# okieraised/rs-face-detection

Hardware: AMD Instinct MI355X
Metric: images/sec + p50 latency, RetinaFace-R50 640x640 b32 (end-to-end detect: preprocess + CNN + decode + NMS; `value` = frames resident in HBM, `value_host_path` = SURVEY 8(d)'s H2D -> ... -> D2H figure) (higher is better)
Workload: dtype bf16; 1 GPU; RetinaFace-ResNet50 640x640 batch=32 bf16 per GPU (BASELINE.json configs[2]); batch_per_gpu=32, global_batch=32, max_det=1024, parallelism=single GPU

## Files before the change

include/rfd.h:

```cpp
#ifndef RFD_H
#define RFD_H

#include <stddef.h>
#include <stdint.h>

#ifdef __cplusplus
extern "C" {
#endif

#define RFD_VERSION 1

#if defined(__GNUC__)
#define RFD_API __attribute__((visibility("default")))
#else
#define RFD_API
#endif

typedef enum rfd_status {
    RFD_OK = 0,
    RFD_ERR_INVALID_ARG = -1,
    RFD_ERR_NO_DEVICE = -2,
    RFD_ERR_HIP = -3,
    RFD_ERR_CAPACITY = -4,
    RFD_ERR_STATE = -5,
// ... 584 lines not shown
                                    const rfd_redact_config *cfg , int32_t *applied , int async);
RFD_API int rfd_redact_faces(rfd_ctx *ctx, const rfd_image *imgs, const rfd_image *dst, int n, const rfd_dets *dets, const uint32_t *sel,
                             const rfd_redact_config *cfg, int32_t *applied);

RFD_API int rfd_get_stats(rfd_ctx *ctx, rfd_stats *stats);
RFD_API int rfd_get_config(const rfd_ctx *ctx, rfd_config *cfg);
RFD_API int rfd_set_thresholds(rfd_ctx *ctx, float confidence_threshold, float iou_threshold);
RFD_API int rfd_set_profiling(rfd_ctx *ctx, int enable);
RFD_API int rfd_get_conv_profile(rfd_ctx *ctx, float *ms_conv, double *flops_conv, int *launches);
RFD_API int rfd_get_op_profile(rfd_ctx *ctx, float *ms, int cap);

RFD_API int rfd_debug_tensor_io(rfd_ctx *ctx, int tensor_id, int n, void *host, int write);
RFD_API int rfd_debug_run_ops(rfd_ctx *ctx, int n, int first_op, int last_op);
RFD_API int rfd_debug_run_chain(rfd_ctx *ctx, int n, int first_op, int last_op, int batch_off, int co_running);
RFD_API int rfd_debug_pass_chains(rfd_ctx *ctx, int n, int *sizes, int cap);
RFD_API int rfd_debug_buffer_io(rfd_ctx *ctx, int tensor_id, void *host, size_t bytes, int write, size_t *image_pitch);
RFD_API int rfd_debug_set_conv_tile(rfd_ctx *ctx, int tile);
RFD_API int rfd_debug_op_kernels(rfd_ctx *ctx, int n, int op, int co_running, char *names, int cap);
RFD_API int rfd_debug_op_kernels_static(int backbone, int net_w, int net_h, int n, int op, int co_running, int tile, int schedule,
                                        int cus, char *names, int cap);
RFD_API int rfd_debug_set_concurrency(rfd_ctx *ctx, int multi_stream, int split_min_part, int split_max_parts,
                                      int use_graph);

RFD_API int rfd_debug_poke_nms_flag(rfd_ctx *ctx, int value);
RFD_API int rfd_debug_align_setup(rfd_ctx *ctx, int n, const float *boxes, const float *kps, const int32_t *found,
                                  const int32_t *img_w, const int32_t *img_h, const rfd_alignment_config *cfg, int32_t *mode,
                                  double *M, int32_t *roi, double *scale, int32_t *area_fast);
RFD_API int rfd_debug_persistent_kernel(int i, const char **name, size_t *lds_bytes);

#ifdef __cplusplus
// ... 4 lines not shown
```

rs-face-detection_amd/csrc/detector.hip:

```cpp
#include <dlfcn.h>
#include <stdarg.h>
#include <stdlib.h>

#include <algorithm>
#include <cmath>
#include <memory>
#include <mutex>
#include <vector>

#include "ctx_access.h"
#include "face_host.h"
#include "frame_host.h"
#include "host_resources.h"
#include "jpeg_encode_host.h"
#include "jpeg_host.h"
#include "network.h"
#include "redact_host.h"
#include "shot_quality_host.h"
#include "view_plan.h"

namespace rfd {

static thread_local char g_err[512] = "";

// ... 151 lines not shown
    JpegEncoder encoder;
    Redact redact;
    struct PipeSlot {
        DevBuf frames, imgs, scale, ob, ol, oc, ot;
        Pinned<PreImage> pin_imgs;
        Pinned<float> pin_scale, h_ob, h_ol;
        Pinned<int> h_oc, h_ot;
        Event h2d, done, post;
        int n = 0;
    };
    static constexpr int kPipe = 2;
    static constexpr int kPipeRows = 128;
    PipeSlot pipe[kPipe];
    int pipe_head = 0, pipe_tail = 0, pipe_inflight = 0;
    DevBuf ov_imgs[2], ov_scale[2];
    Event ov_chain_done[2][2], ov_post_done[2], ov_desc;
    bool ov_post_valid[2] = {false, false};
    int ov_parity = 0;
    int ov_last_n = -1;
    Event ov_resync;
    Rccl::Comm comm = nullptr;
    int comm_rank = 0, comm_world = 0;
    rfd_stats stats;
    float conv_ms = 0.f;
    double conv_flops = 0.0;
    int conv_launches = 0;

    int ensure_network()
    {
        if (net_created) return RFD_OK;
        RFD_TRY(net.create(cfg.backbone, cfg.image_w, cfg.image_h, cfg.max_batch_size, cfg.precision, cfg.schedule));
// ... 229 lines not shown
        c->conv_ms = 0.f; c->conv_flops = 0.0; c->conv_launches = 0;
        for (size_t i = 0; i < c->net.g.ops.size(); ++i)
            if (c->net.g.ops[i].kind == OP_CONV || c->net.g.ops[i].kind == OP_B2B) {
                c->conv_ms += c->net.op_ms[i];
                c->conv_flops += 2.0 * c->net.g.layer_macs((int)i) * n;
                ++c->conv_launches;
            }
    }
    return RFD_OK;
}

int detect_overlapped(rfd_ctx *c, const rfd_image *imgs, int n, rfd_dets *out, hipEvent_t frames_ready = nullptr)
{
    Network &net = c->net;
    RFD_TRY(net.ensure_alt_heads());
    const size_t B = (size_t)c->cfg.max_batch_size;
    if (!c->ov_desc) {
        RFD_TRY(c->ov_desc.create());
        RFD_TRY(c->ov_resync.create());
        for (int a = 0; a < 2; ++a) {
            RFD_TRY(c->ov_post_done[a].create());
            for (int b = 0; b < 2; ++b) RFD_TRY(c->ov_chain_done[a][b].create());
            RFD_TRY(c->ov_imgs[a].reserve(B * sizeof(PreImage)));
            RFD_TRY(c->ov_scale[a].reserve(B * sizeof(float)));
        }
    }
    const int par = (c->ov_parity ^= 1);
    PreImage *pis;
    float *pin_scales;
    RFD_TRY(acquire_frame_slot(c, &pis, &pin_scales));
    for (int i = 0; i < n; ++i) RFD_TRY(fill_pre_image(c, imgs[i], i, &pis[i], &pin_scales[i]));
    RFD_TRY(place_frames(c, imgs, n, true, pis, sizeof *pis));
    hipStream_t st[2] = {net.part_stream[0], net.part_stream[1]};
    if (c->ov_last_n != n) {
        RFD_HIP(hipEventRecord(c->ov_resync, c->stream));
        for (int p = 0; p < 2; ++p) RFD_HIP(hipStreamWaitEvent(st[p], c->ov_resync, 0));
    }
    c->ov_last_n = n;
    if (frames_ready)
        for (int p = 0; p < 2; ++p) RFD_HIP(hipStreamWaitEvent(st[p], frames_ready, 0));
    if (c->ov_post_valid[par])
        for (int p = 0; p < 2; ++p) RFD_HIP(hipStreamWaitEvent(st[p], c->ov_post_done[par], 0));
    RFD_HIP(hipMemcpyAsync(c->ov_imgs[par].p, pis, n * sizeof(PreImage), hipMemcpyHostToDevice, st[0]));
    RFD_HIP(hipMemcpyAsync(c->ov_scale[par].p, pin_scales, n * sizeof(float), hipMemcpyHostToDevice, st[0]));
    RFD_TRY(c->frame_ring.record(st[0]));
    RFD_HIP(hipEventRecord(c->ov_desc, st[0]));
    RFD_HIP(hipStreamWaitEvent(st[1], c->ov_desc, 0));
    net.head_parity = par;
    net.co_running = 1;
    int chain[Network::kMaxParts];
    if (net.pass_chains(n, chain) != 2) { set_error("overlapped calls run as two chains"); return RFD_ERR_STATE; }
    const int B0 = chain[0];
    int status = RFD_OK;
    for (int p = 0; p < 2 && status == RFD_OK; ++p) {
        const int off = p ? B0 : 0, Bp = chain[p];
        status = launch_preprocess(pre_params(c, (const PreImage *)c->ov_imgs[par].p + off, off), Bp, st[p]);
        if (status == RFD_OK) status = net.run(Bp, st[p], 0, -1, off, p);
        if (status == RFD_OK && hipEventRecord(c->ov_chain_done[par][p], st[p]) != hipSuccess) status = RFD_ERR_HIP;
    }
    net.co_running = 0;
    if (status != RFD_OK) { net.head_parity = 0; c->ov_last_n = -1; return status; }
    for (int p = 0; p < 2; ++p) RFD_HIP(hipStreamWaitEvent(c->stream, c->ov_chain_done[par][p], 0));
    DecodeParams dp = decode_params(c, true);
    net.head_parity = 0;
    RFD_TRY(post_network(c, dp, false, n, out->boxes, out->landmarks, out->count, out->total, nullptr,
                         (const float *)c->ov_scale[par].p));
    RFD_HIP(hipEventRecord(c->ov_post_done[par], c->stream));
    c->ov_post_valid[par] = true;
    return RFD_OK;
}

int detect_impl(rfd_ctx *c, const rfd_image *imgs, int n, rfd_dets *out, bool on_device, int async, bool frames_on_device)
{
    RFD_CHECK_ARG(c != nullptr, "ctx is null");
    RFD_CHECK_ARG(out && out->boxes && out->landmarks && out->count, "output buffers are null");
    RFD_TRY(check_images(c, imgs, n));
    RFD_TRY(c->ensure_network());
    if (!c->net.weights_ready) { set_error("network weights are not initialised"); return RFD_ERR_STATE; }
    if (async == 2 && on_device && frames_on_device && !c->net.profiling && c->net.multi_stream && c->net.num_parts(n) == 2) {
// ... 910 lines not shown
    RFD_HIP(hipSetDevice(c->cfg.device_id));
    const float *scales;
    RFD_TRY(stage_frames(c, imgs, n, false, &scales));
    const size_t npix = (size_t)n * c->cfg.image_h * c->cfg.image_w;
    PreParams pp = pre_params(c, c->imgs.p, -1);
    if (det_img) { RFD_TRY(c->scratch[0].reserve(npix * 3)); pp.out_det_img = (uint8_t *)c->scratch[0].p; }
    if (tensor) { RFD_TRY(c->scratch[1].reserve(npix * 3 * sizeof(float))); pp.out_tensor = (float *)c->scratch[1].p; }
    RFD_TRY(launch_preprocess(pp, n, c->stream));
    if (det_img) RFD_HIP(hipMemcpyAsync(det_img, pp.out_det_img, npix * 3, hipMemcpyDeviceToHost, c->stream));
    if (tensor) RFD_HIP(hipMemcpyAsync(tensor, pp.out_tensor, npix * 3 * sizeof(float), hipMemcpyDeviceToHost, c->stream));
    RFD_HIP(hipStreamSynchronize(c->stream));
    if (det_scale) memcpy(det_scale, scales, n * sizeof(float));
    return RFD_OK;
}

int rfd_forward(rfd_ctx *c, const float *tensor, int n, float *const heads[9])
{
    RFD_CHECK_ARG(c && tensor && heads, "null argument");
    for (int i = 0; i < 9; ++i) RFD_CHECK_ARG(heads[i] != nullptr, "head pointer is null");
    RFD_TRY(check_batch(c, n, "batch"));
    RFD_HIP(hipSetDevice(c->cfg.device_id));
    RFD_TRY(c->ensure_network());
    c->ov_last_n = -1;
    const size_t plane = (size_t)c->cfg.image_h * c->cfg.image_w;
    RFD_TRY(c->scratch[1].reserve(n * plane * 3 * sizeof(float)));
    RFD_HIP(hipMemcpyAsync(c->scratch[1].p, tensor, n * plane * 3 * sizeof(float), hipMemcpyHostToDevice, c->stream));
    RFD_TRY(launch_tensor_to_nhwc4((const float *)c->scratch[1].p, (bf16_t *)c->net.tensor_ptr(c->net.g.input), n,
                                   c->cfg.image_h, c->cfg.image_w, c->stream));
    RFD_TRY(c->net.run(n, c->stream));
    RFD_HIP(hipMemcpyAsync(c->h_nms_flag, c->net.d_fail, sizeof(int), hipMemcpyDeviceToHost, c->stream));
// ... 295 lines not shown
```

rs-face-detection_amd/csrc/kernels_pre.hip:

```cpp
#include "kernels.h"

namespace rfd {

__device__ __forceinline__ int coef11(float v)
{
    int r = __float2int_rn(v);
    return max(-32768, min(32767, r));
}

__device__ __forceinline__ void resize_linear_px(const uint8_t *src, long long stride, int h, int w, double scale_x,
                                                 double scale_y, int area_fast, int x, int y, int v[3])
{
    if (area_fast) {
        const uint8_t *s0 = src + (long long)(2 * y) * stride + 2 * x * 3;
        const uint8_t *s1 = s0 + stride;
#pragma unroll
        for (int c = 0; c < 3; ++c) v[c] = (s0[c] + s0[c + 3] + s1[c] + s1[c + 3] + 2) >> 2;
        return;
    }
    float fx = (float)(((double)x + 0.5) * scale_x - 0.5);
    int sx = (int)floorf(fx);
    fx -= (float)sx;
    if (sx < 0) { fx = 0.0f; sx = 0; }
    if (sx >= w - 1) { fx = 0.0f; sx = w - 1; }
    const int a0 = coef11((1.0f - fx) * 2048.0f), a1 = coef11(fx * 2048.0f);
    const int sx1 = min(sx + 1, w - 1);

    float fy = (float)(((double)y + 0.5) * scale_y - 0.5);
    const int sy = (int)floorf(fy);
    fy -= (float)sy;
    const int b0 = coef11((1.0f - fy) * 2048.0f), b1 = coef11(fy * 2048.0f);
    const int sy0 = min(max(sy, 0), h - 1), sy1 = min(max(sy + 1, 0), h - 1);
    const uint8_t *S0 = src + (long long)sy0 * stride;
    const uint8_t *S1 = src + (long long)sy1 * stride;
    typedef uint64_t u64_unaligned __attribute__((aligned(1)));
    int t0[6], t1[6];
    const long long o0 = (long long)sy0 * stride + sx * 3, o1 = (long long)sy1 * stride + sx * 3, lim = (long long)(h - 1) * stride + (long long)w * 3 - 8;
    if (sx1 == sx + 1 && o0 <= lim && o1 <= lim) {
        const uint64_t q0 = *reinterpret_cast<const u64_unaligned *>(src + o0), q1 = *reinterpret_cast<const u64_unaligned *>(src + o1);
#pragma unroll
        for (int k = 0; k < 6; ++k) { t0[k] = (int)((q0 >> (8 * k)) & 0xff); t1[k] = (int)((q1 >> (8 * k)) & 0xff); }
    } else {
#pragma unroll
        for (int c = 0; c < 3; ++c) { t0[c] = S0[sx * 3 + c]; t0[3 + c] = S0[sx1 * 3 + c]; t1[c] = S1[sx * 3 + c]; t1[3 + c] = S1[sx1 * 3 + c]; }
    }
#pragma unroll
    for (int c = 0; c < 3; ++c) {
        const int r0 = t0[c] * a0 + t0[3 + c] * a1;
        const int r1 = t1[c] * a0 + t1[3 + c] * a1;
        v[c] = (((b0 * (r0 >> 4)) >> 16) + ((b1 * (r1 >> 4)) >> 16) + 2) >> 2;
        v[c] = min(255, max(0, v[c]));
    }
}

__global__ void __launch_bounds__(256) preprocess_kernel(PreParams p)
{
    const int b = blockIdx.z;
    const int x = blockIdx.x * 64 + (threadIdx.x & 63);
    const int y = blockIdx.y * 4 + (threadIdx.x >> 6);
    if (x >= p.net_w || y >= p.net_h) return;
    const PreImage im = p.imgs[b];

    int v[3] = {0, 0, 0};
    if (x < im.new_w && y < im.new_h) resize_linear_px(im.src, im.stride, im.h, im.w, im.scale_x, im.scale_y, im.area_fast, x, y, v);
    const size_t pix = ((size_t)b * p.net_h + y) * p.net_w + x;
    if (p.out_nhwc4) {
        const uint32_t r = __float_as_uint((float)v[2]) >> 16, g = __float_as_uint((float)v[1]) >> 16;
        const uint32_t bl = __float_as_uint((float)v[0]) >> 16;
        uint2 o;
        o.x = r | (g << 16);
        o.y = bl;
        *reinterpret_cast<uint2 *>(p.out_nhwc4 + pix * 4) = o;
    }
    if (p.out_det_img) {
        uint8_t *d = p.out_det_img + pix * 3;
        d[0] = (uint8_t)v[0]; d[1] = (uint8_t)v[1]; d[2] = (uint8_t)v[2];
    }
    if (p.out_tensor) {
        const size_t plane = (size_t)p.net_h * p.net_w;
        float *t = p.out_tensor + (size_t)b * 3 * plane + (size_t)y * p.net_w + x;
        t[0] = ((float)v[2] / 1.0f - 0.0f) / 1.0f;
        t[plane] = ((float)v[1] / 1.0f - 0.0f) / 1.0f;
        t[2 * plane] = ((float)v[0] / 1.0f - 0.0f) / 1.0f;
    }
}

int launch_preprocess(const PreParams &p, int n, hipStream_t s)
{
    dim3 grid(ceil_div(p.net_w, 64), ceil_div(p.net_h, 4), n);
    hipLaunchKernelGGL(preprocess_kernel, grid, dim3(256), 0, s, p);
    RFD_HIP(hipGetLastError());
    return RFD_OK;
}

__device__ __forceinline__ uint32_t f32_to_bf16_bits(float f)
{
    uint32_t u = __float_as_uint(f);
    if ((u & 0x7fffffffu) > 0x7f800000u) return (u >> 16) | 0x40u;
    u += 0x7fffu + ((u >> 16) & 1u);
    return u >> 16;
}

__global__ void __launch_bounds__(256) tensor_to_nhwc4_kernel(const float *__restrict__ t,
                                                              bf16_t *__restrict__ out, size_t plane,
// ... 511 lines not shown
```

rs-face-detection_amd/csrc/network.h:

```cpp
#pragma once
#include <string>
#include <vector>

#include "kernels.h"

namespace rfd {

enum LayerKind { LK_CONV = 0, LK_DEPTHWISE = 1, LK_FIRST3X3 = 2, LK_CONV0 = 3 };

struct Layer {
    std::string name;
    int cin, cout, kh, kw, stride, pad;
    int kind;
    int cin_d, cout_d;
    int has_affine;
    float gain;
    size_t w_off;
    size_t ldw;
    size_t w_elems;
    size_t b_off;
    size_t a_off;
};

enum OpKind { OP_CONV = 2, OP_STEM = 3, OP_DW = 4, OP_FIRST = 5, OP_B2B = 6 };
// ... 95 lines not shown
    size_t sk_ws_bytes[3] = {0, 0, 0};
    unsigned *d_sk_cnt = nullptr;
    std::vector<int> sk_cnt_off, sk_cnt_n;
    bool latency_pass(int B) const { return schedule == RFD_SCHEDULE_LATENCY && precision == 0 && B >= 1 && B <= RFD_LATENCY_MAX_BATCH; }
    int create(int backbone, int net_w, int net_h, int max_batch, int precision = 0, int schedule = 0);
    void destroy();
    int init_synthetic(uint64_t seed, hipStream_t s);
    int get_layer(int idx, float *w, float *bias, hipStream_t s);
    int set_layer(int idx, const float *w, const float *bias, hipStream_t s);
    int get_affine(int idx, float *scale, float *shift, hipStream_t s);
    int set_affine(int idx, const float *scale, const float *shift, hipStream_t s);
    void *tensor_ptr(int t, int batch_off = 0) const
    {
        const int bi = g.tensors[t].buffer;
        void *base = (head_parity && bi < (int)d_alt.size() && d_alt[bi]) ? d_alt[bi] : d_buffers[bi];
        return (char *)base + (size_t)batch_off * g.buffer_bytes_per_image[bi];
    }
    std::vector<void *> d_alt;
    int head_parity = 0;
    int ensure_alt_heads();
    void op_launch(int i, int B, int batch_off, int part, bool offer_conv1, OpLaunch *out) const;
    int op_kernel_names(int n, int op, int cus, std::string *out) const;
    int plan_splitk();
    int run(int B, hipStream_t s, int first_op = 0, int last_op = -1, int batch_off = 0, int part = 0);
    int run_split(int B, hipStream_t s);
    int split_body(int B, hipStream_t s);
    int tune_streams(int B, int P, hipStream_t s);
    void assign_streams(int a, int b, int c);
    static constexpr int kPool = 8;
    hipStream_t pool[kPool] = {};
    bool tuned = false, tune = true;
    float tuned_ms = 0.f;
    int tuned_a = -1, tuned_b = -1;
    int run_graphed(int B, hipStream_t s);
    std::vector<hipGraphExec_t> graph_exec;
    std::vector<char> warmed;
    bool use_graph = true;
    static constexpr int kMaxParts = 4;
    hipStream_t side[kMaxParts][2] = {};
    hipEvent_t ev_fork[kMaxParts][2] = {}, ev_join[kMaxParts][2] = {};
    bool multi_stream = true;
    hipStream_t part_stream[kMaxParts] = {};
    hipEvent_t ev_part_fork = nullptr, ev_part_join[kMaxParts] = {};
    int co_running = 0;
    int split_min_part = 4;
    int split_max_parts = 2;
    int num_parts(int B) const
    {
        if (profiling || split_min_part < 1 || precision != 0 || latency_pass(B)) return 1;
        return std::max(1, std::min(std::min(split_max_parts, kMaxParts), B / split_min_part));
    }
    int pass_chains(int B, int *sizes) const
    {
        const int P = num_parts(B);
        for (int p = 0; p < P; ++p) sizes[p] = B / P + (p < B % P ? 1 : 0);
        return P;
    }
// ... 5 lines not shown
```

rs-face-detection_amd/csrc/network.hip:

```cpp
#include "network.h"

#include <math.h>
#include <algorithm>
#include <utility>

namespace rfd {

int Graph::add_tensor(int C, int H, int W, int f32)
{
    TensorDesc t;
    t.C_logical = C;
    t.C = (f32 || C == 4 || C % 64 == 0) ? C : (C + 63) / 64 * 64;
    t.H = H; t.W = W; t.is_f32 = f32; t.buffer = -1; t.first = 1 << 30; t.last = -1;
    tensors.push_back(t);
    return (int)tensors.size() - 1;
}

int Graph::add_layer(const std::string &name, int cin, int cout, int k, int stride, int pad, float gain,
                     int has_affine, int extra_k, int parent, int col_off, int kind, int cout_dev)
{
    Layer L;
    L.name = name; L.cin = cin; L.cout = cout; L.kh = k; L.kw = k; L.stride = stride; L.pad = pad;
    L.gain = gain; L.has_affine = has_affine; L.kind = kind;
    L.cin_d = kind == LK_CONV ? (cin + 63) / 64 * 64 : cin;
// ... 421 lines not shown
        if (d_sk_ws[b]) (void)hipFree(d_sk_ws[b]);
        d_sk_ws[b] = nullptr; sk_ws_bytes[b] = 0;
    }
    if (d_sk_cnt) (void)hipFree(d_sk_cnt);
    d_sk_cnt = nullptr;
    if (d_stem32) (void)hipFree(d_stem32);
    d_stem32 = nullptr;
    for (void *p : d_buffers32)
        if (p) (void)hipFree(p);
    d_buffers32.clear();
    for (void *p : d_buffers)
        if (p) (void)hipFree(p);
    for (void *p : d_alt)
        if (p) (void)hipFree(p);
    d_alt.clear();
    for (int hh = 0; hh < kMaxParts; ++hh) {
        for (int i = 0; i < 2; ++i) {
            if (ev_fork[hh][i]) (void)hipEventDestroy(ev_fork[hh][i]);
            if (ev_join[hh][i]) (void)hipEventDestroy(ev_join[hh][i]);
            side[hh][i] = nullptr; ev_fork[hh][i] = ev_join[hh][i] = nullptr;
        }
        if (ev_part_join[hh]) (void)hipEventDestroy(ev_part_join[hh]);
        part_stream[hh] = nullptr; ev_part_join[hh] = nullptr;
    }
    for (int i = 0; i < kPool; ++i) {
        if (pool[i]) (void)hipStreamDestroy(pool[i]);
        pool[i] = nullptr;
    }
    if (ev_part_fork) (void)hipEventDestroy(ev_part_fork);
    ev_part_fork = nullptr;
// ... 500 lines not shown
}

int Network::ensure_alt_heads()
{
    if (!d_alt.empty()) return RFD_OK;
    d_alt.assign(d_buffers.size(), nullptr);
    for (int l = 0; l < 3; ++l) {
        const int bi = g.tensors[g.heads[l]].buffer;
        RFD_HIP(hipMalloc(&d_alt[bi], g.buffer_bytes_per_image[bi] * (size_t)max_batch));
        RFD_HIP(hipMemset(d_alt[bi], 0, g.buffer_bytes_per_image[bi] * (size_t)max_batch));
    }
    RFD_HIP(hipDeviceSynchronize());
    return RFD_OK;
}

void Network::assign_streams(int a, int b, int c)
{
    part_stream[0] = pool[a];
    part_stream[1] = pool[b];
    if (c >= 0) part_stream[2] = pool[c];
    int k = 0;
    auto next = [&]() {
        while (k == a || k == b || k == c) ++k;
        return pool[k++ % kPool];
    };
    const int nchain = c >= 0 ? 3 : 2;
    for (int hh = 0; hh < nchain; ++hh)
        for (int i = 0; i < 2; ++i) side[hh][i] = next();
    for (int hh = nchain; hh < kMaxParts; ++hh) {
        part_stream[hh] = next();
        for (int i = 0; i < 2; ++i) side[hh][i] = next();
    }
}


int Network::split_body(int B, hipStream_t s)
{
    int sizes[kMaxParts];
    const int P = pass_chains(B, sizes);
    RFD_HIP(hipEventRecord(ev_part_fork, s));
    co_running = 1;
    int off = 0, st = RFD_OK;
    for (int p = 0; p < P && st == RFD_OK; ++p) {
// ... 126 lines not shown
```

rs-face-detection_amd/python/rfd_hip/__init__.py:

```python
import ctypes as C
import os

import numpy as np

_HERE = os.path.dirname(os.path.abspath(__file__))
LIB_PATH = os.path.normpath(os.path.join(_HERE, "..", "..", "librfd_hip.so"))

RFD_OK = 0
RFD_ERR_INVALID_ARG = -1
RFD_ERR_NO_DEVICE = -2
PRECISION_BF16, PRECISION_F32 = 0, 1
SCHEDULE_THROUGHPUT, SCHEDULE_LATENCY = 0, 1
LATENCY_MAX_BATCH = 2
RFD_ERR_HIP = -3
RFD_ERR_CAPACITY = -4
RFD_ERR_STATE = -5
RFD_ERR_IO = -6
RFD_ERR_COMM = -7
RFD_ERR_UNSUPPORTED = -8
JPEG_GRAY, JPEG_444, JPEG_422, JPEG_420 = 0, 1, 2, 3
JPEG_ENTROPY_HOST, JPEG_ENTROPY_DEVICE = 0, 1
JPEG_PATH_HOST, JPEG_PATH_DEVICE, JPEG_PATH_REFUSED = 0, 1, 2
JPEG_ORIENTATION_IGNORE, JPEG_ORIENTATION_APPLY = 0, 1
COMM_ID_BYTES = 128
# ... 200 lines not shown

class rfd_tensor_desc(C.Structure):
    _fields_ = [("channels", C.c_int), ("height", C.c_int), ("width", C.c_int),
                ("is_f32", C.c_int), ("buffer", C.c_int), ("is_input", C.c_int),
                ("head_level", C.c_int), ("channels_logical", C.c_int), ("reserved", C.c_int * 3)]


API_SYMBOLS = [
    "rfd_config_default", "rfd_create", "rfd_destroy", "rfd_last_error", "rfd_version",
    "rfd_graph_create", "rfd_graph_destroy", "rfd_graph_counts", "rfd_graph_layer", "rfd_graph_op",
    "rfd_graph_tensor", "rfd_graph_macs", "rfd_graph_workspace_bytes",
    "rfd_init_synthetic_weights", "rfd_num_layers", "rfd_get_layer_weights",
    "rfd_set_layer_weights", "rfd_get_layer_affine", "rfd_set_layer_affine", "rfd_detect_batch",
    "rfd_detect_batch_device", "rfd_sync", "rfd_set_stream", "rfd_preprocess", "rfd_forward", "rfd_decode_nms",
    "rfd_nms_sorted", "_nms", "rfd_get_stats", "rfd_get_config", "rfd_set_thresholds", "rfd_set_profiling",
    "rfd_get_conv_profile", "rfd_get_op_profile", "rfd_debug_tensor_io", "rfd_debug_run_ops", "rfd_debug_run_chain", "rfd_debug_pass_chains", "rfd_debug_buffer_io",
    "rfd_debug_set_conv_tile", "rfd_debug_op_kernels", "rfd_debug_op_kernels_static", "rfd_debug_set_concurrency", "rfd_debug_persistent_kernel", "rfd_debug_poke_nms_flag", "rfd_selection_config_default",
    "rfd_select_faces", "rfd_detect_select_batch", "rfd_save_weights", "rfd_load_weights",
    "rfd_alignment_config_default", "rfd_align_faces", "rfd_detect_select_align_batch", "rfd_debug_align_setup",
    "rfd_host_alloc", "rfd_host_free", "rfd_submit_batch", "rfd_collect_batch",
    "rfd_comm_get_unique_id", "rfd_comm_init", "rfd_comm_info", "rfd_gather_detections", "rfd_comm_destroy",
    "rfd_face_tensor_config_quality", "rfd_face_tensor_config_extraction", "rfd_face_tensors",
    "rfd_align_faces_tensors", "rfd_detect_select_align_tensors_batch", "rfd_detect_faces_device", "rfd_quality_decide", "rfd_normalize_embeddings",
    "rfd_quality_decide_device", "rfd_normalize_embeddings_device",
    "rfd_face_tensor_config_quality_assessment", "rfd_liveness_config_default", "rfd_liveness_tensors",
    "rfd_liveness_tensors_device", "rfd_liveness_decide", "rfd_liveness_decide_device",
    "rfd_gallery_create", "rfd_gallery_destroy", "rfd_gallery_size", "rfd_gallery_clear", "rfd_gallery_add", "rfd_gallery_add_device",
    "rfd_gallery_get_rows", "rfd_gallery_search", "rfd_gallery_search_device", "rfd_debug_gallery_offset",
    "rfd_gallery_remove", "rfd_gallery_replace", "rfd_gallery_replace_device", "rfd_gallery_live", "rfd_gallery_removed",
    "rfd_gallery_save", "rfd_gallery_load", "rfd_gallery_file_info",
    "rfd_gallery_set_identities", "rfd_gallery_get_identities", "rfd_gallery_identities", "rfd_gallery_search_identities",
# ... 64 lines not shown
    L.rfd_forward.argtypes = [vp, vp, ci, C.POINTER(vp)]
    L.rfd_decode_nms.argtypes = [vp, C.POINTER(vp), ci, vp, C.POINTER(rfd_dets), vp]
    L.rfd_nms_sorted.argtypes = [vp, vp, C.POINTER(ci), vp, ci, ci, C.c_float]
    L._nms.argtypes = [vp, C.POINTER(ci), vp, ci, ci, C.c_float, ci]
    L._nms.restype = None
    L.rfd_get_stats.argtypes = [vp, C.POINTER(rfd_stats)]
    L.rfd_get_config.argtypes = [vp, C.POINTER(rfd_config)]
    L.rfd_set_thresholds.argtypes = [vp, C.c_float, C.c_float]
    L.rfd_set_profiling.argtypes = [vp, ci]
    L.rfd_get_conv_profile.argtypes = [vp, C.POINTER(C.c_float), C.POINTER(C.c_double), C.POINTER(ci)]
    L.rfd_get_op_profile.argtypes = [vp, vp, ci]
    L.rfd_debug_tensor_io.argtypes = [vp, ci, ci, vp, ci]
    L.rfd_debug_run_ops.argtypes = [vp, ci, ci, ci]
    L.rfd_debug_run_chain.argtypes = [vp, ci, ci, ci, ci, ci]
    L.rfd_debug_pass_chains.argtypes = [vp, ci, C.POINTER(ci), ci]
    L.rfd_debug_buffer_io.argtypes = [vp, ci, vp, C.c_size_t, ci, C.POINTER(C.c_size_t)]
    L.rfd_debug_set_conv_tile.argtypes = [vp, ci]
    L.rfd_debug_set_concurrency.argtypes = [vp, ci, ci, ci, ci]
    L.rfd_debug_op_kernels.argtypes = [vp, ci, ci, ci, C.c_char_p, ci]
    L.rfd_debug_op_kernels_static.argtypes = [ci] * 9 + [C.c_char_p, ci]
    L.rfd_debug_poke_nms_flag.argtypes = [vp, ci]
    L.rfd_debug_persistent_kernel.argtypes = [ci, C.POINTER(C.c_char_p), C.POINTER(C.c_size_t)]
    L.rfd_save_weights.argtypes = [vp, C.c_char_p]
    L.rfd_load_weights.argtypes = [vp, C.c_char_p]
    L.rfd_selection_config_default.argtypes = [vp]
    L.rfd_selection_config_default.restype = None
    L.rfd_select_faces.argtypes = [vp, C.POINTER(rfd_dets), vp, vp, ci, vp, ci, vp, vp, vp]
    L.rfd_detect_select_batch.argtypes = [vp, C.POINTER(rfd_image), ci, vp, ci, vp, vp, vp]
    L.rfd_host_alloc.argtypes = [C.c_size_t, C.POINTER(C.c_void_p)]
    L.rfd_host_free.argtypes = [vp]
# ... 1711 lines not shown

    def debug_set_concurrency(self, multi_stream=True, split_min_part=8, split_max_parts=2, use_graph=True):
        _check(self._L.rfd_debug_set_concurrency(self._ctx, int(multi_stream), int(split_min_part), int(split_max_parts),
                                                 int(use_graph)))

    def debug_run(self, n, first_op, last_op, batch_off=0, co_running=False):
        if batch_off == 0 and not co_running:
            _check(self._L.rfd_debug_run_ops(self._ctx, n, first_op, last_op))
        else:
            _check(self._L.rfd_debug_run_chain(self._ctx, n, first_op, last_op, batch_off, 1 if co_running else 0))

    def debug_pass_chains(self, n):
        sizes = (C.c_int * 8)()
        return list(sizes[:_check(self._L.rfd_debug_pass_chains(self._ctx, n, sizes, 8))])

    def debug_buffer_pitch(self, tensor_id):
        pitch = C.c_size_t()
        _check(self._L.rfd_debug_buffer_io(self._ctx, tensor_id, None, 0, 0, C.byref(pitch)))
        return pitch.value

    def debug_buffer_read(self, tensor_id):
        a = np.zeros(self.cfg.max_batch_size * self.debug_buffer_pitch(tensor_id), np.uint8)
        _check(self._L.rfd_debug_buffer_io(self._ctx, tensor_id, a.ctypes.data, a.nbytes, 0, None))
        return a

    def debug_buffer_write(self, tensor_id, arr):
        a = np.ascontiguousarray(arr).reshape(-1).view(np.uint8)
        _check(self._L.rfd_debug_buffer_io(self._ctx, tensor_id, a.ctypes.data, a.nbytes, 1, None))

    def stats(self):
# ... 20 lines not shown
```

Measured before the change: 7881 images/s.

## Run preprocess on a dedicated stream with double-buffered input and vectorize resize

In the overlapped detect path, preprocessing moves from the two chain streams to a separate pre-stream that writes into a parity-alternated input buffer. The next batch's preprocess can then overlap the current CNN chains, and both chains wait on one event. The preprocess kernel also handles four pixels per thread, using wide unaligned 64-bit source loads and vectorized stores. This cuts per-pixel load and store instructions but requires the canvas width to be a multiple of four. A debug API for canvas preprocessing is added as well.

New measurement: 7880 images/s. About the same (-0.0%).

```diff
diff --git a/include/rfd.h b/include/rfd.h
--- a/include/rfd.h
+++ b/include/rfd.h
@@ -622,6 +622,8 @@
 RFD_API int rfd_debug_run_ops(rfd_ctx *ctx, int n, int first_op, int last_op);
 RFD_API int rfd_debug_run_chain(rfd_ctx *ctx, int n, int first_op, int last_op, int batch_off, int co_running);
 RFD_API int rfd_debug_pass_chains(rfd_ctx *ctx, int n, int *sizes, int cap);
+RFD_API int rfd_debug_preprocess_canvas(rfd_ctx *ctx, const rfd_image *imgs, int n, int frames_on_device, int canvas_w, int canvas_h,
+                                uint8_t *det_img, float *tensor, uint16_t *nhwc4);
 RFD_API int rfd_debug_buffer_io(rfd_ctx *ctx, int tensor_id, void *host, size_t bytes, int write, size_t *image_pitch);
 RFD_API int rfd_debug_set_conv_tile(rfd_ctx *ctx, int tile);
 RFD_API int rfd_debug_op_kernels(rfd_ctx *ctx, int n, int op, int co_running, char *names, int cap);
diff --git a/rs-face-detection_amd/csrc/detector.hip b/rs-face-detection_amd/csrc/detector.hip
--- a/rs-face-detection_amd/csrc/detector.hip
+++ b/rs-face-detection_amd/csrc/detector.hip
@@ -189,7 +189,7 @@
     PipeSlot pipe[kPipe];
     int pipe_head = 0, pipe_tail = 0, pipe_inflight = 0;
     DevBuf ov_imgs[2], ov_scale[2];
-    Event ov_chain_done[2][2], ov_post_done[2], ov_desc;
+    Event ov_chain_done[2][2], ov_post_done[2], ov_pre_done[2];
     bool ov_post_valid[2] = {false, false};
     int ov_parity = 0;
     int ov_last_n = -1;
@@ -449,12 +449,13 @@
 {
     Network &net = c->net;
     RFD_TRY(net.ensure_alt_heads());
+    RFD_TRY(net.ensure_alt_input());
     const size_t B = (size_t)c->cfg.max_batch_size;
-    if (!c->ov_desc) {
-        RFD_TRY(c->ov_desc.create());
+    if (!c->ov_resync) {
         RFD_TRY(c->ov_resync.create());
         for (int a = 0; a < 2; ++a) {
             RFD_TRY(c->ov_post_done[a].create());
+            RFD_TRY(c->ov_pre_done[a].create());
             for (int b = 0; b < 2; ++b) RFD_TRY(c->ov_chain_done[a][b].create());
             RFD_TRY(c->ov_imgs[a].reserve(B * sizeof(PreImage)));
             RFD_TRY(c->ov_scale[a].reserve(B * sizeof(float)));
@@ -466,38 +467,43 @@
     RFD_TRY(acquire_frame_slot(c, &pis, &pin_scales));
     for (int i = 0; i < n; ++i) RFD_TRY(fill_pre_image(c, imgs[i], i, &pis[i], &pin_scales[i]));
     RFD_TRY(place_frames(c, imgs, n, true, pis, sizeof *pis));
-    hipStream_t st[2] = {net.part_stream[0], net.part_stream[1]};
+    hipStream_t st[2] = {net.part_stream[0], net.part_stream[1]}, pre = net.pre_stream;
     if (c->ov_last_n != n) {
         RFD_HIP(hipEventRecord(c->ov_resync, c->stream));
-        for (int p = 0; p < 2; ++p) RFD_HIP(hipStreamWaitEvent(st[p], c->ov_resync, 0));
+        RFD_HIP(hipStreamWaitEvent(pre, c->ov_resync, 0));
     }
     c->ov_last_n = n;
     if (frames_ready)
-        for (int p = 0; p < 2; ++p) RFD_HIP(hipStreamWaitEvent(st[p], frames_ready, 0));
-    if (c->ov_post_valid[par])
-        for (int p = 0; p < 2; ++p) RFD_HIP(hipStreamWaitEvent(st[p], c->ov_post_done[par], 0));
-    RFD_HIP(hipMemcpyAsync(c->ov_imgs[par].p, pis, n * sizeof(PreImage), hipMemcpyHostToDevice, st[0]));
-    RFD_HIP(hipMemcpyAsync(c->ov_scale[par].p, pin_scales, n * sizeof(float), hipMemcpyHostToDevice, st[0]));
-    RFD_TRY(c->frame_ring.record(st[0]));
-    RFD_HIP(hipEventRecord(c->ov_desc, st[0]));
-    RFD_HIP(hipStreamWaitEvent(st[1], c->ov_desc, 0));
-    net.head_parity = par;
+        RFD_HIP(hipStreamWaitEvent(pre, frames_ready, 0));
+    if (c->ov_post_valid[par]) RFD_HIP(hipStreamWaitEvent(pre, c->ov_post_done[par], 0));
+    RFD_HIP(hipMemcpyAsync(c->ov_imgs[par].p, pis, n * sizeof(PreImage), hipMemcpyHostToDevice, pre));
+    RFD_HIP(hipMemcpyAsync(c->ov_scale[par].p, pin_scales, n * sizeof(float), hipMemcpyHostToDevice, pre));
+    RFD_TRY(c->frame_ring.record(pre));
+    net.head_parity = net.input_parity = par;
     net.co_running = 1;
     int chain[Network::kMaxParts];
-    if (net.pass_chains(n, chain) != 2) { set_error("overlapped calls run as two chains"); return RFD_ERR_STATE; }
+    int status = RFD_OK;
+    if (net.pass_chains(n, chain) != 2) { set_error("overlapped calls run as two chains"); status = RFD_ERR_STATE; }
+    if (status == RFD_OK) status = launch_preprocess(pre_params(c, c->ov_imgs[par].p, 0), n, pre);
+    if (status == RFD_OK && hipEventRecord(c->ov_pre_done[par], pre) != hipSuccess) status = RFD_ERR_HIP;
     const int B0 = chain[0];
-    int status = RFD_OK;
     for (int p = 0; p < 2 && status == RFD_OK; ++p) {
         const int off = p ? B0 : 0, Bp = chain[p];
-        status = launch_preprocess(pre_params(c, (const PreImage *)c->ov_imgs[par].p + off, off), Bp, st[p]);
+        if (hipStreamWaitEvent(st[p], c->ov_pre_done[par], 0) != hipSuccess) status = RFD_ERR_HIP;
         if (status == RFD_OK) status = net.run(Bp, st[p], 0, -1, off, p);
         if (status == RFD_OK && hipEventRecord(c->ov_chain_done[par][p], st[p]) != hipSuccess) status = RFD_ERR_HIP;
     }
     net.co_running = 0;
-    if (status != RFD_OK) { net.head_parity = 0; c->ov_last_n = -1; return status; }
+    if (status != RFD_OK) {
+        (void)hipStreamSynchronize(pre);
+        for (int p = 0; p < 2; ++p) (void)hipStreamSynchronize(st[p]);
+        net.head_parity = net.input_parity = 0;
+        c->ov_last_n = -1;
+        return status;
+    }
     for (int p = 0; p < 2; ++p) RFD_HIP(hipStreamWaitEvent(c->stream, c->ov_chain_done[par][p], 0));
     DecodeParams dp = decode_params(c, true);
-    net.head_parity = 0;
+    net.head_parity = net.input_parity = 0;
     RFD_TRY(post_network(c, dp, false, n, out->boxes, out->landmarks, out->count, out->total, nullptr,
                          (const float *)c->ov_scale[par].p));
     RFD_HIP(hipEventRecord(c->ov_post_done[par], c->stream));
@@ -1438,6 +1444,42 @@
     return RFD_OK;
 }
 
+int rfd_debug_preprocess_canvas(rfd_ctx *c, const rfd_image *imgs, int n, int frames_on_device, int canvas_w, int canvas_h,
+                                uint8_t *det_img, float *tensor, uint16_t *nhwc4)
+{
+    RFD_CHECK_ARG(c != nullptr, "ctx is null");
+    RFD_CHECK_ARG(canvas_w > 0 && canvas_h > 0, "the canvas is empty");
+    RFD_TRY(check_images(c, imgs, n));
+    RFD_HIP(hipSetDevice(c->cfg.device_id));
+    PreImage *pis;
+    float *pin_scales;
+    RFD_TRY(acquire_frame_slot(c, &pis, &pin_scales));
+    for (int i = 0; i < n; ++i) {
+        letterbox(imgs[i].height, imgs[i].width, canvas_w, canvas_h, &pis[i], &pin_scales[i]);
+        if (pis[i].new_w <= 0 || pis[i].new_h <= 0) {
+            set_error("invalid argument: frame %d (%dx%d) letterboxes to an empty %dx%d image", i, imgs[i].width, imgs[i].height, pis[i].new_w, pis[i].new_h);
+            return RFD_ERR_INVALID_ARG;
+        }
+    }
+    RFD_TRY(place_frames(c, imgs, n, frames_on_device != 0, pis, sizeof *pis));
+    RFD_HIP(hipMemcpyAsync(c->imgs.p, pis, n * sizeof(PreImage), hipMemcpyHostToDevice, c->stream));
+    RFD_TRY(c->frame_ring.record(c->stream));
+    const size_t npix = (size_t)n * canvas_h * canvas_w;
+    PreParams pp;
+    memset(&pp, 0, sizeof pp);
+    pp.imgs = (const PreImage *)c->imgs.p;
+    pp.net_h = canvas_h; pp.net_w = canvas_w;
+    if (det_img) { RFD_TRY(c->scratch[0].reserve(npix * 3)); pp.out_det_img = (uint8_t *)c->scratch[0].p; }
+    if (tensor) { RFD_TRY(c->scratch[1].reserve(npix * 3 * sizeof(float))); pp.out_tensor = (float *)c->scratch[1].p; }
+    if (nhwc4) { RFD_TRY(c->scratch[2].reserve(npix * 4 * sizeof(uint16_t))); pp.out_nhwc4 = (bf16_t *)c->scratch[2].p; }
+    RFD_TRY(launch_preprocess(pp, n, c->stream));
+    if (det_img) RFD_HIP(hipMemcpyAsync(det_img, pp.out_det_img, npix * 3, hipMemcpyDeviceToHost, c->stream));
+    if (tensor) RFD_HIP(hipMemcpyAsync(tensor, pp.out_tensor, npix * 3 * sizeof(float), hipMemcpyDeviceToHost, c->stream));
+    if (nhwc4) RFD_HIP(hipMemcpyAsync(nhwc4, pp.out_nhwc4, npix * 4 * sizeof(uint16_t), hipMemcpyDeviceToHost, c->stream));
+    RFD_HIP(hipStreamSynchronize(c->stream));
+    return RFD_OK;
+}
+
 int rfd_forward(rfd_ctx *c, const float *tensor, int n, float *const heads[9])
 {
     RFD_CHECK_ARG(c && tensor && heads, "null argument");
diff --git a/rs-face-detection_amd/csrc/kernels_pre.hip b/rs-face-detection_amd/csrc/kernels_pre.hip
--- a/rs-face-detection_amd/csrc/kernels_pre.hip
+++ b/rs-face-detection_amd/csrc/kernels_pre.hip
@@ -6,6 +6,35 @@
 {
     int r = __float2int_rn(v);
     return max(-32768, min(32767, r));
+}
+
+__device__ __forceinline__ void linear_taps_x(int x, double scale_x, int w, int &sx, int &a0, int &a1)
+{
+    float fx = (float)(((double)x + 0.5) * scale_x - 0.5);
+    sx = (int)floorf(fx);
+    fx -= (float)sx;
+    if (sx < 0) { fx = 0.0f; sx = 0; }
+    if (sx >= w - 1) { fx = 0.0f; sx = w - 1; }
+    a0 = coef11((1.0f - fx) * 2048.0f);
+    a1 = coef11(fx * 2048.0f);
+}
+
+__device__ __forceinline__ void linear_taps_y(int y, double scale_y, int h, int &sy0, int &sy1, int &b0, int &b1)
+{
+    float fy = (float)(((double)y + 0.5) * scale_y - 0.5);
+    const int sy = (int)floorf(fy);
+    fy -= (float)sy;
+    b0 = coef11((1.0f - fy) * 2048.0f);
+    b1 = coef11(fy * 2048.0f);
+    sy0 = min(max(sy, 0), h - 1);
+    sy1 = min(max(sy + 1, 0), h - 1);
+}
+
+__device__ __forceinline__ int linear_mix(int p0, int p1, int q0, int q1, int a0, int a1, int b0, int b1)
+{
+    const int r0 = p0 * a0 + p1 * a1;
+    const int r1 = q0 * a0 + q1 * a1;
+    return min(255, max(0, (((b0 * (r0 >> 4)) >> 16) + ((b1 * (r1 >> 4)) >> 16) + 2) >> 2));
 }
 
 __device__ __forceinline__ void resize_linear_px(const uint8_t *src, long long stride, int h, int w, double scale_x,
@@ -18,19 +47,10 @@
         for (int c = 0; c < 3; ++c) v[c] = (s0[c] + s0[c + 3] + s1[c] + s1[c + 3] + 2) >> 2;
         return;
     }
-    float fx = (float)(((double)x + 0.5) * scale_x - 0.5);
-    int sx = (int)floorf(fx);
-    fx -= (float)sx;
-    if (sx < 0) { fx = 0.0f; sx = 0; }
-    if (sx >= w - 1) { fx = 0.0f; sx = w - 1; }
-    const int a0 = coef11((1.0f - fx) * 2048.0f), a1 = coef11(fx * 2048.0f);
+    int sx, a0, a1, sy0, sy1, b0, b1;
+    linear_taps_x(x, scale_x, w, sx, a0, a1);
     const int sx1 = min(sx + 1, w - 1);
-
-    float fy = (float)(((double)y + 0.5) * scale_y - 0.5);
-    const int sy = (int)floorf(fy);
-    fy -= (float)sy;
-    const int b0 = coef11((1.0f - fy) * 2048.0f), b1 = coef11(fy * 2048.0f);
-    const int sy0 = min(max(sy, 0), h - 1), sy1 = min(max(sy + 1, 0), h - 1);
+    linear_taps_y(y, scale_y, h, sy0, sy1, b0, b1);
     const uint8_t *S0 = src + (long long)sy0 * stride;
     const uint8_t *S1 = src + (long long)sy1 * stride;
     typedef uint64_t u64_unaligned __attribute__((aligned(1)));
@@ -45,49 +65,125 @@
         for (int c = 0; c < 3; ++c) { t0[c] = S0[sx * 3 + c]; t0[3 + c] = S0[sx1 * 3 + c]; t1[c] = S1[sx * 3 + c]; t1[3 + c] = S1[sx1 * 3 + c]; }
     }
 #pragma unroll
-    for (int c = 0; c < 3; ++c) {
-        const int r0 = t0[c] * a0 + t0[3 + c] * a1;
-        const int r1 = t1[c] * a0 + t1[3 + c] * a1;
-        v[c] = (((b0 * (r0 >> 4)) >> 16) + ((b1 * (r1 >> 4)) >> 16) + 2) >> 2;
-        v[c] = min(255, max(0, v[c]));
-    }
-}
+    for (int c = 0; c < 3; ++c) v[c] = linear_mix(t0[c], t0[3 + c], t1[c], t1[3 + c], a0, a1, b0, b1);
+}
+
+__device__ __forceinline__ uint64_t window_bytes(uint64_t q0, uint64_t q1, uint64_t q2, int d)
+{
+    const int i = d >> 3, s = (d & 7) * 8;
+    const uint64_t lo = i == 0 ? q0 : (i == 1 ? q1 : q2);
+    const uint64_t hi = i == 0 ? q1 : (i == 1 ? q2 : 0);
+    return s ? (lo >> s) | (hi << (64 - s)) : lo;
+}
+
+__device__ __forceinline__ int byte_of(uint64_t u, int k) { return (int)((u >> (8 * k)) & 0xff); }
+
+constexpr int kPreGroup = 4;
 
 __global__ void __launch_bounds__(256) preprocess_kernel(PreParams p)
 {
-    const int b = blockIdx.z;
-    const int x = blockIdx.x * 64 + (threadIdx.x & 63);
-    const int y = blockIdx.y * 4 + (threadIdx.x >> 6);
-    if (x >= p.net_w || y >= p.net_h) return;
+    const int b = blockIdx.y;
+    const int groups_w = p.net_w / kPreGroup;
+    const int g = blockIdx.x * 256 + threadIdx.x;
+    if (g >= groups_w * p.net_h) return;
+    const int y = g / groups_w, x0 = (g - y * groups_w) * kPreGroup;
     const PreImage im = p.imgs[b];
 
-    int v[3] = {0, 0, 0};
-    if (x < im.new_w && y < im.new_h) resize_linear_px(im.src, im.stride, im.h, im.w, im.scale_x, im.scale_y, im.area_fast, x, y, v);
-    const size_t pix = ((size_t)b * p.net_h + y) * p.net_w + x;
+    int v[kPreGroup][3];
+#pragma unroll
+    for (int k = 0; k < kPreGroup; ++k) v[k][0] = v[k][1] = v[k][2] = 0;
+    const int nv = y < im.new_h ? min(kPreGroup, im.new_w - x0) : 0;
+    if (nv > 0) {
+        typedef uint64_t u64_unaligned __attribute__((aligned(1)));
+        const long long extent = (long long)(im.h - 1) * im.stride + (long long)im.w * 3;
+        bool done = false;
+        if (im.area_fast) {
+            const long long o0 = (long long)(2 * y) * im.stride + (long long)x0 * 6, o1 = o0 + im.stride;
+            if (o1 + 24 <= extent) {
+                const u64_unaligned *r0 = reinterpret_cast<const u64_unaligned *>(im.src + o0);
+                const u64_unaligned *r1 = reinterpret_cast<const u64_unaligned *>(im.src + o1);
+                const uint64_t q00 = r0[0], q01 = r0[1], q02 = r0[2], q10 = r1[0], q11 = r1[1], q12 = r1[2];
+#pragma unroll
+                for (int k = 0; k < kPreGroup; ++k) {
+                    const uint64_t u0 = window_bytes(q00, q01, q02, 6 * k), u1 = window_bytes(q10, q11, q12, 6 * k);
+#pragma unroll
+                    for (int c = 0; c < 3; ++c)
+                        if (k < nv) v[k][c] = (byte_of(u0, c) + byte_of(u0, c + 3) + byte_of(u1, c) + byte_of(u1, c + 3) + 2) >> 2;
+                }
+                done = true;
+            }
+        } else {
+            int sy0, sy1, b0, b1, sx[kPreGroup], a0[kPreGroup], a1[kPreGroup];
+            linear_taps_y(y, im.scale_y, im.h, sy0, sy1, b0, b1);
+#pragma unroll
+            for (int k = 0; k < kPreGroup; ++k) linear_taps_x(x0 + min(k, nv - 1), im.scale_x, im.w, sx[k], a0[k], a1[k]);
+            const int span = sx[kPreGroup - 1] - sx[0];
+            const int need = span * 3 + 6 <= 16 ? 16 : 24;
+            const long long o0 = (long long)sy0 * im.stride + (long long)sx[0] * 3, o1 = (long long)sy1 * im.stride + (long long)sx[0] * 3;
+            if (span * 3 + 6 <= 24 && max(o0, o1) + need <= extent) {
+                const u64_unaligned *r0 = reinterpret_cast<const u64_unaligned *>(im.src + o0);
+                const u64_unaligned *r1 = reinterpret_cast<const u64_unaligned *>(im.src + o1);
+                const uint64_t q00 = r0[0], q01 = r0[1], q10 = r1[0], q11 = r1[1];
+                uint64_t q02 = 0, q12 = 0;
+                if (need == 24) { q02 = r0[2]; q12 = r1[2]; }
+#pragma unroll
+                for (int k = 0; k < kPreGroup; ++k) {
+                    const int d = (sx[k] - sx[0]) * 3;
+                    const uint64_t u0 = window_bytes(q00, q01, q02, d), u1 = window_bytes(q10, q11, q12, d);
+#pragma unroll
+                    for (int c = 0; c < 3; ++c)
+                        if (k < nv) v[k][c] = linear_mix(byte_of(u0, c), byte_of(u0, c + 3), byte_of(u1, c), byte_of(u1, c + 3), a0[k], a1[k], b0, b1);
+                }
+                done = true;
+            }
+        }
+        if (!done) {
+#pragma unroll
+            for (int k = 0; k < kPreGroup; ++k)
+                if (k < nv) resize_linear_px(im.src, im.stride, im.h, im.w, im.scale_x, im.scale_y, im.area_fast, x0 + k, y, v[k]);
+        }
+    }
+    const size_t pix = ((size_t)b * p.net_h + y) * p.net_w + x0;
     if (p.out_nhwc4) {
-        const uint32_t r = __float_as_uint((float)v[2]) >> 16, g = __float_as_uint((float)v[1]) >> 16;
-        const uint32_t bl = __float_as_uint((float)v[0]) >> 16;
-        uint2 o;
-        o.x = r | (g << 16);
-        o.y = bl;
-        *reinterpret_cast<uint2 *>(p.out_nhwc4 + pix * 4) = o;
+        uint32_t w[kPreGroup][2];
+#pragma unroll
+        for (int k = 0; k < kPreGroup; ++k) {
+            w[k][0] = (__float_as_uint((float)v[k][2]) >> 16) | ((__float_as_uint((float)v[k][1]) >> 16) << 16);
+            w[k][1] = __float_as_uint((float)v[k][0]) >> 16;
+        }
+        uint4 *o = reinterpret_cast<uint4 *>(p.out_nhwc4 + pix * 4);
+        o[0] = make_uint4(w[0][0], w[0][1], w[1][0], w[1][1]);
+        o[1] = make_uint4(w[2][0], w[2][1], w[3][0], w[3][1]);
     }
     if (p.out_det_img) {
-        uint8_t *d = p.out_det_img + pix * 3;
-        d[0] = (uint8_t)v[0]; d[1] = (uint8_t)v[1]; d[2] = (uint8_t)v[2];
+        uint32_t *d = reinterpret_cast<uint32_t *>(p.out_det_img + pix * 3);
+        d[0] = (uint32_t)v[0][0] | ((uint32_t)v[0][1] << 8) | ((uint32_t)v[0][2] << 16) | ((uint32_t)v[1][0] << 24);
+        d[1] = (uint32_t)v[1][1] | ((uint32_t)v[1][2] << 8) | ((uint32_t)v[2][0] << 16) | ((uint32_t)v[2][1] << 24);
+        d[2] = (uint32_t)v[2][2] | ((uint32_t)v[3][0] << 8) | ((uint32_t)v[3][1] << 16) | ((uint32_t)v[3][2] << 24);
     }
     if (p.out_tensor) {
         const size_t plane = (size_t)p.net_h * p.net_w;
-        float *t = p.out_tensor + (size_t)b * 3 * plane + (size_t)y * p.net_w + x;
-        t[0] = ((float)v[2] / 1.0f - 0.0f) / 1.0f;
-        t[plane] = ((float)v[1] / 1.0f - 0.0f) / 1.0f;
-        t[2 * plane] = ((float)v[0] / 1.0f - 0.0f) / 1.0f;
+        float *t = p.out_tensor + (size_t)b * 3 * plane + (size_t)y * p.net_w + x0;
+#pragma unroll
+        for (int ch = 0; ch < 3; ++ch) {
+            float4 o;
+            o.x = ((float)v[0][2 - ch] / 1.0f - 0.0f) / 1.0f;
+            o.y = ((float)v[1][2 - ch] / 1.0f - 0.0f) / 1.0f;
+            o.z = ((float)v[2][2 - ch] / 1.0f - 0.0f) / 1.0f;
+            o.w = ((float)v[3][2 - ch] / 1.0f - 0.0f) / 1.0f;
+            *reinterpret_cast<float4 *>(t + ch * plane) = o;
+        }
     }
 }
 
 int launch_preprocess(const PreParams &p, int n, hipStream_t s)
 {
-    dim3 grid(ceil_div(p.net_w, 64), ceil_div(p.net_h, 4), n);
+    static_assert(kPreGroup == 4, "the stores of preprocess_kernel are written for groups of four pixels");
+    if (p.net_w < kPreGroup || p.net_w % kPreGroup != 0 || p.net_h < 1) {
+        set_error("invalid argument: the canvas must be a multiple of %d pixels wide (%dx%d)", kPreGroup, p.net_w, p.net_h);
+        return RFD_ERR_INVALID_ARG;
+    }
+    dim3 grid(ceil_div(p.net_w / kPreGroup * p.net_h, 256), n);
     hipLaunchKernelGGL(preprocess_kernel, grid, dim3(256), 0, s, p);
     RFD_HIP(hipGetLastError());
     return RFD_OK;
diff --git a/rs-face-detection_amd/csrc/network.h b/rs-face-detection_amd/csrc/network.h
--- a/rs-face-detection_amd/csrc/network.h
+++ b/rs-face-detection_amd/csrc/network.h
@@ -133,11 +133,15 @@
     {
         const int bi = g.tensors[t].buffer;
         void *base = (head_parity && bi < (int)d_alt.size() && d_alt[bi]) ? d_alt[bi] : d_buffers[bi];
+        if (input_parity && t == g.input && d_alt_input) base = d_alt_input;
         return (char *)base + (size_t)batch_off * g.buffer_bytes_per_image[bi];
     }
     std::vector<void *> d_alt;
     int head_parity = 0;
     int ensure_alt_heads();
+    void *d_alt_input = nullptr;
+    int input_parity = 0;
+    int ensure_alt_input();
     void op_launch(int i, int B, int batch_off, int part, bool offer_conv1, OpLaunch *out) const;
     int op_kernel_names(int n, int op, int cus, std::string *out) const;
     int plan_splitk();
@@ -160,6 +164,7 @@
     hipEvent_t ev_fork[kMaxParts][2] = {}, ev_join[kMaxParts][2] = {};
     bool multi_stream = true;
     hipStream_t part_stream[kMaxParts] = {};
+    hipStream_t pre_stream = nullptr;
     hipEvent_t ev_part_fork = nullptr, ev_part_join[kMaxParts] = {};
     int co_running = 0;
     int split_min_part = 4;
diff --git a/rs-face-detection_amd/csrc/network.hip b/rs-face-detection_amd/csrc/network.hip
--- a/rs-face-detection_amd/csrc/network.hip
+++ b/rs-face-detection_amd/csrc/network.hip
@@ -459,6 +459,10 @@
     for (void *p : d_alt)
         if (p) (void)hipFree(p);
     d_alt.clear();
+    if (d_alt_input) (void)hipFree(d_alt_input);
+    d_alt_input = nullptr;
+    head_parity = input_parity = 0;
+    pre_stream = nullptr;
     for (int hh = 0; hh < kMaxParts; ++hh) {
         for (int i = 0; i < 2; ++i) {
             if (ev_fork[hh][i]) (void)hipEventDestroy(ev_fork[hh][i]);
@@ -989,6 +993,16 @@
     return RFD_OK;
 }
 
+int Network::ensure_alt_input()
+{
+    if (d_alt_input) return RFD_OK;
+    const size_t bytes = g.buffer_bytes_per_image[g.tensors[g.input].buffer] * (size_t)max_batch;
+    RFD_HIP(hipMalloc(&d_alt_input, bytes));
+    RFD_HIP(hipMemset(d_alt_input, 0, bytes));
+    RFD_HIP(hipDeviceSynchronize());
+    return RFD_OK;
+}
+
 void Network::assign_streams(int a, int b, int c)
 {
     part_stream[0] = pool[a];
@@ -1002,6 +1016,11 @@
     const int nchain = c >= 0 ? 3 : 2;
     for (int hh = 0; hh < nchain; ++hh)
         for (int i = 0; i < 2; ++i) side[hh][i] = next();
+    {
+        int kp = k;
+        while (kp == a || kp == b || kp == c) ++kp;
+        pre_stream = pool[kp % kPool];
+    }
     for (int hh = nchain; hh < kMaxParts; ++hh) {
         part_stream[hh] = next();
         for (int i = 0; i < 2; ++i) side[hh][i] = next();
diff --git a/rs-face-detection_amd/python/rfd_hip/__init__.py b/rs-face-detection_amd/python/rfd_hip/__init__.py
--- a/rs-face-detection_amd/python/rfd_hip/__init__.py
+++ b/rs-face-detection_amd/python/rfd_hip/__init__.py
@@ -238,7 +238,7 @@
     "rfd_set_layer_weights", "rfd_get_layer_affine", "rfd_set_layer_affine", "rfd_detect_batch",
     "rfd_detect_batch_device", "rfd_sync", "rfd_set_stream", "rfd_preprocess", "rfd_forward", "rfd_decode_nms",
     "rfd_nms_sorted", "_nms", "rfd_get_stats", "rfd_get_config", "rfd_set_thresholds", "rfd_set_profiling",
-    "rfd_get_conv_profile", "rfd_get_op_profile", "rfd_debug_tensor_io", "rfd_debug_run_ops", "rfd_debug_run_chain", "rfd_debug_pass_chains", "rfd_debug_buffer_io",
+    "rfd_get_conv_profile", "rfd_get_op_profile", "rfd_debug_tensor_io", "rfd_debug_run_ops", "rfd_debug_run_chain", "rfd_debug_pass_chains", "rfd_debug_preprocess_canvas", "rfd_debug_buffer_io",
     "rfd_debug_set_conv_tile", "rfd_debug_op_kernels", "rfd_debug_op_kernels_static", "rfd_debug_set_concurrency", "rfd_debug_persistent_kernel", "rfd_debug_poke_nms_flag", "rfd_selection_config_default",
     "rfd_select_faces", "rfd_detect_select_batch", "rfd_save_weights", "rfd_load_weights",
     "rfd_alignment_config_default", "rfd_align_faces", "rfd_detect_select_align_batch", "rfd_debug_align_setup",
@@ -333,6 +333,7 @@
     L.rfd_debug_run_ops.argtypes = [vp, ci, ci, ci]
     L.rfd_debug_run_chain.argtypes = [vp, ci, ci, ci, ci, ci]
     L.rfd_debug_pass_chains.argtypes = [vp, ci, C.POINTER(ci), ci]
+    L.rfd_debug_preprocess_canvas.argtypes = [vp, C.POINTER(rfd_image), ci, ci, ci, ci, vp, vp, vp]
     L.rfd_debug_buffer_io.argtypes = [vp, ci, vp, C.c_size_t, ci, C.POINTER(C.c_size_t)]
     L.rfd_debug_set_conv_tile.argtypes = [vp, ci]
     L.rfd_debug_set_concurrency.argtypes = [vp, ci, ci, ci, ci]
@@ -2074,6 +2075,23 @@
         sizes = (C.c_int * 8)()
         return list(sizes[:_check(self._L.rfd_debug_pass_chains(self._ctx, n, sizes, 8))])
 
+    def debug_preprocess_canvas(self, frames, canvas, device_frames=None):
+        if device_frames is None:
+            arr, keep = self._images(frames)
+            n = len(frames)
+        else:
+            n = len(device_frames)
+            arr = (rfd_image * n)()
+            for i, (ptr, h, w, stride) in enumerate(device_frames):
+                arr[i].data, arr[i].height, arr[i].width, arr[i].stride = ptr, h, w, stride
+        w, h = canvas
+        det_img = np.zeros((n, h, w, 3), np.uint8)
+        tensor = np.zeros((n, 3, h, w), np.float32)
+        nhwc4 = np.zeros((n, h, w, 4), np.uint16)
+        _check(self._L.rfd_debug_preprocess_canvas(self._ctx, arr, n, int(device_frames is not None), w, h, det_img.ctypes.data,
+                                                   tensor.ctypes.data, nhwc4.ctypes.data))
+        return det_img, tensor, nhwc4
+
     def debug_buffer_pitch(self, tensor_id):
         pitch = C.c_size_t()
         _check(self._L.rfd_debug_buffer_io(self._ctx, tensor_id, None, 0, 0, C.byref(pitch)))
```
